# tontinton/dbeel

Hardware: AMD Instinct MI355X
Metric: compaction_MBps_input (higher is better)
Workload: dtype u8; 1 GPU; cfg3_8run_x_1GiB; n_runs=8, entries_per_run=987000, key_size=32, keep_tombstones=False, parallelism=independent_jobs_x1

## Files before the change

dbeel_amd/csrc/dbeel_gpu.hip:

```cpp
#include <cstdarg>
#include <cstdint>
#include <cstdio>
#include <cstring>
#include <cstdlib>
#include <new>
#include <vector>

#include <hip/hip_runtime.h>
#include <rocprim/rocprim.hpp>

#include "../../include/dbeel_gpu.h"

#define MAX_RUNS 64

static thread_local char g_err[512];

static void set_err(const char* fmt, ...) {
    va_list ap;
    va_start(ap, fmt);
    vsnprintf(g_err, sizeof g_err, fmt, ap);
    va_end(ap);
}

extern "C" const char* dbeel_gpu_last_error(void) { return g_err; }
// ... 113 lines not shown


#define DERR_CORRUPT 1u
#define DERR_UNSORTED 2u

__device__ __forceinline__ uint64_t key_prefix(const uint8_t* key,
                                               uint64_t klen) {
    uint64_t v = 0;
    if (klen >= 8) {
        v = ld_u64(key);
    } else {
        for (uint64_t j = 0; j < klen; j++) v |= (uint64_t)key[j] << (8 * j);
    }
    return __builtin_bswap64(v);
}

template <int KB, bool TS> struct AuxT;
template <int KB> struct AuxT<KB, false> {
    uint8_t key[KB];
    uint32_t klen;
};
template <int KB> struct AuxT<KB, true> {
    uint8_t key[KB];
    uint32_t klen;
    uint32_t rsv;
    uint64_t ts_lo;
    int64_t ts_hi;
};
static_assert(sizeof(AuxT<12, false>) == 16, "tier-0 aux must be 16B");
static_assert(sizeof(AuxT<24, true>) == 48, "tier-1 aux must be 48B");
static_assert(sizeof(AuxT<40, true>) == 64, "tier-2 aux must be 64B");

template <int KB, bool TS>
__device__ __forceinline__ int cmp_keys_sfx(const RunsDesc& R,
                                            const AuxT<KB, TS>* aux, int rA,
                                            uint64_t iA, int rB,
                                            uint64_t iB) {
    const AuxT<KB, TS>* a = aux + R.entry_base[rA] + iA;
    const AuxT<KB, TS>* b = aux + R.entry_base[rB] + iB;
    uint32_t la = a->klen, lb = b->klen;
    uint32_t n = la < lb ? la : lb;
    uint32_t ns = n > 8 ? n - 8 : 0;
    if (ns > KB) ns = KB;
    #pragma unroll
    for (uint32_t i = 0; i < KB; i += 8) {
        if (i >= ns) break;
        uint64_t va, vb;
        __builtin_memcpy(&va, a->key + i, 8);
        __builtin_memcpy(&vb, b->key + i, 8);
        if (i + 8 > ns) {
            uint64_t mask = (~0ull) >> (8 * (i + 8 - ns));
            va &= mask;
            vb &= mask;
        }
        if (va != vb) {
            va = __builtin_bswap64(va);
            vb = __builtin_bswap64(vb);
            return va < vb ? -1 : 1;
        }
    }
    if (la > (uint32_t)(8 + KB) && lb > (uint32_t)(8 + KB)) {
        EView ea, eb;
        if (!load_entry(R, rA, iA, ea) || !load_entry(R, rB, iB, eb))
            return -1;
        return cmp_keys(ea.key, ea.klen, eb.key, eb.klen);
    }
    return la < lb ? -1 : (la > lb ? 1 : 0);
}

__device__ __forceinline__ int cmp_ts_run_blob(const RunsDesc& R, int rA,
                                               uint64_t iA, int rB,
                                               uint64_t iB) {
    EView a, b;
    if (!load_entry(R, rA, iA, a) || !load_entry(R, rB, iB, b))
        return rA < rB ? -1 : 1;
    uint64_t alo, blo;
    int64_t ahi, bhi;
    load_ts(a, alo, ahi);
    load_ts(b, blo, bhi);
    if (ahi != bhi) return ahi < bhi ? -1 : 1;
    if (alo != blo) return alo < blo ? -1 : 1;
    return rA < rB ? -1 : (rA > rB ? 1 : 0);
}

template <int KB, bool TS>
__device__ __forceinline__ int cmp_sfx_full(const RunsDesc& R,
                                            const AuxT<KB, TS>* aux, int rA,
                                            uint64_t iA, int rB,
                                            uint64_t iB) {
    int c = cmp_keys_sfx<KB, TS>(R, aux, rA, iA, rB, iB);
    if (c) return c;
    if constexpr (TS) {
        const AuxT<KB, TS>* a = aux + R.entry_base[rA] + iA;
        const AuxT<KB, TS>* b = aux + R.entry_base[rB] + iB;
        if (a->ts_hi != b->ts_hi) return a->ts_hi < b->ts_hi ? -1 : 1;
        if (a->ts_lo != b->ts_lo) return a->ts_lo < b->ts_lo ? -1 : 1;
        return rA < rB ? -1 : (rA > rB ? 1 : 0);
    } else {
        return cmp_ts_run_blob(R, rA, iA, rB, iB);
    }
}

template <int KB, bool TS>
__global__ void k_prepare(RunsDesc R, uint64_t g0, uint64_t g1,
                          uint64_t* pfx, AuxT<KB, TS>* aux, uint32_t* err) {
    uint64_t stride = (uint64_t)gridDim.x * blockDim.x;
    for (uint64_t g = g0 + (uint64_t)blockIdx.x * blockDim.x + threadIdx.x;
         g < g1; g += stride) {
        int r = 0;
        while (r + 1 < R.n_runs && g >= R.entry_base[r + 1]) r++;
        uint64_t i = g - R.entry_base[r];
        EView e;
        if (!load_entry(R, r, i, e)) {
            atomicOr(err, DERR_CORRUPT);
            pfx[g] = 0;
            AuxT<KB, TS> z = {};
            aux[g] = z;
            continue;
        }
        pfx[g] = key_prefix(e.key, e.klen);
        AuxT<KB, TS> a;
        a.klen = (uint32_t)e.klen;
        if constexpr (TS) {
            a.rsv = 0;
            load_ts(e, a.ts_lo, a.ts_hi);
        }
        uint32_t nk = e.klen > 8 ? (uint32_t)e.klen - 8 : 0;
        if (nk > KB) nk = KB;
        if (nk >= KB) {
            #pragma unroll
            for (uint32_t j = 0; j < KB; j += 8) {
                uint64_t v = ld_u64(e.key + 8 + j);
                uint32_t nb = (KB - j) < 8 ? (KB - j) : 8;
                __builtin_memcpy(a.key + j, &v, nb);
            }
        } else {
            #pragma unroll
            for (uint32_t j = 0; j < KB; j += 8) {
                uint64_t v = 0;
                if (j < nk) {
                    v = ld_u64(e.key + 8 + j);
                    if (j + 8 > nk)
                        v &= (~0ull) >> (8 * (j + 8 - nk));
                }
                uint32_t nb = (KB - j) < 8 ? (KB - j) : 8;
                __builtin_memcpy(a.key + j, &v, nb);
            }
        }
        aux[g] = a;
        if (ld_u64(e.raw) != e.klen ||
            ld_u64(e.raw + 8 + e.klen) != (uint64_t)e.full_size - 32 - e.klen)
            atomicOr(err, DERR_CORRUPT);
        if (i + 1 < R.count[r]) {
            uint64_t noff = ld_u64(R.index[r] + (i + 1) * 16);
            if (e.off + e.full_size > noff)
                atomicOr(err, DERR_CORRUPT);
        }
    }
}


#define CORANK_BLOCK 256
#define CORANK_STEPS 8
#define CORANK_BLOCK_POS (CORANK_BLOCK * CORANK_STEPS)
#define CR_LOSER 0x80000000u
#define CR_MASK 0x7FFFFFFFu

struct PairDesc {
    uint32_t a, b;
    uint64_t chunk_base;
};

template <int KB, bool TS>
__global__ void k_corners(RunsDesc R, const uint64_t* pfx,
                          const AuxT<KB, TS>* aux, const PairDesc* pairs,
                          uint32_t n_pairs, uint64_t total_chunks,
                          uint64_t* corners) {
    uint64_t stride = (uint64_t)gridDim.x * blockDim.x;
    for (uint64_t t = (uint64_t)blockIdx.x * blockDim.x + threadIdx.x;
         t < total_chunks; t += stride) {
        uint32_t plo = 0, phi = n_pairs;
        while (plo < phi) {
            uint32_t mid = (plo + phi) >> 1;
            if (pairs[mid].chunk_base <= t)
                plo = mid + 1;
            else
                phi = mid;
        }
        const PairDesc P = pairs[plo - 1];
        const int a = (int)P.a, b = (int)P.b;
        const uint64_t Na = R.count[a], Nb = R.count[b];
        const uint64_t* gpa = pfx + R.entry_base[a];
        const uint64_t* gpb = pfx + R.entry_base[b];
        uint64_t diag = (t - P.chunk_base) * CORANK_BLOCK_POS;
        uint64_t slo = diag > Nb ? diag - Nb : 0;
        uint64_t shi = diag < Na ? diag : Na;
        while (slo < shi) {
            uint64_t mid = (slo + shi) >> 1;
            uint64_t pa = gpa[mid], pb = gpb[diag - mid - 1];
            int c = (pa != pb)
                        ? (pa < pb ? -1 : 1)
                        : cmp_sfx_full<KB, TS>(R, aux, a, mid, b,
                                               diag - mid - 1);
            if (c < 0)
                slo = mid + 1;
            else
                shi = mid;
        }
        corners[t] = slo;
    }
}

template <int KB, bool TS, int BLK = CORANK_BLOCK>
__global__ __launch_bounds__(BLK) void k_corank(
    RunsDesc R, const uint64_t* pfx, const AuxT<KB, TS>* aux,
    const PairDesc* pairs, uint32_t n_pairs, uint64_t total_chunks,
    const uint64_t* corners, uint32_t* cr) {
    constexpr int STEPS = CORANK_BLOCK_POS / BLK;
    __shared__ uint64_t s_pfx[CORANK_BLOCK_POS + 2];
    __shared__ uint32_t s_cr[CORANK_BLOCK_POS];
    for (uint64_t t = blockIdx.x; t < total_chunks; t += gridDim.x) {
        uint32_t plo = 0, phi = n_pairs;
        while (plo < phi) {
            uint32_t mid = (plo + phi) >> 1;
            if (pairs[mid].chunk_base <= t)
                plo = mid + 1;
            else
                phi = mid;
        }
        uint64_t pair_end_chunk =
            (plo < n_pairs) ? pairs[plo].chunk_base : total_chunks;
        const PairDesc P = pairs[plo - 1];
        const int a = (int)P.a, b = (int)P.b;
        const uint64_t Na = R.count[a], Nb = R.count[b];
        const uint64_t* gpa = pfx + R.entry_base[a];
        const uint64_t* gpb = pfx + R.entry_base[b];
        uint64_t diag0 = (t - P.chunk_base) * CORANK_BLOCK_POS;
        uint64_t diag1 = diag0 + CORANK_BLOCK_POS;
        if (diag1 > Na + Nb) diag1 = Na + Nb;

        const uint64_t iaS = corners[t];
        const uint64_t ibS = diag0 - iaS;
        const uint64_t iaE = (t + 1 < pair_end_chunk) ? corners[t + 1] : Na;
        const uint64_t ibE = diag1 - iaE;
        const uint32_t lenA = (uint32_t)(iaE - iaS);
        const uint32_t lenB = (uint32_t)(ibE - ibS);

        for (uint32_t u = threadIdx.x; u < lenA; u += BLK)
            s_pfx[u] = gpa[iaS + u];
        for (uint32_t u = threadIdx.x; u < lenB; u += BLK)
            s_pfx[lenA + u] = gpb[ibS + u];
        __syncthreads();
        const uint64_t* sA = s_pfx;
        const uint64_t* sB = s_pfx + lenA;

        uint32_t L = lenA + lenB;
        uint32_t d = threadIdx.x * STEPS;
        if (d < L) {
            uint32_t slo = d > lenB ? d - lenB : 0;
            uint32_t shi = d < lenA ? d : lenA;
            while (slo < shi) {
                uint32_t mid = (slo + shi) >> 1;
                uint64_t pa = sA[mid], pb = sB[d - mid - 1];
                int c = (pa != pb) ? (pa < pb ? -1 : 1)
                                   : cmp_sfx_full<KB, TS>(R, aux, a, iaS + mid,
                                                          b, ibS + d - mid - 1);
                if (c < 0)
                    slo = mid + 1;
                else
                    shi = mid;
            }
            uint32_t ja = slo, jb = d - slo;
            uint32_t dend = d + STEPS;
            if (dend > L) dend = L;

            for (uint32_t pos = d; pos < dend; pos++) {
                bool take_a;
                if (ja >= lenA)
                    take_a = false;
                else if (jb >= lenB)
                    take_a = true;
                else {
                    uint64_t pa = sA[ja], pb = sB[jb];
                    take_a = (pa != pb)
                                 ? (pa < pb)
                                 : (cmp_sfx_full<KB, TS>(R, aux, a, iaS + ja, b,
                                                         ibS + jb) < 0);
                }
                if (take_a) {
                    uint64_t gib = ibS + jb;
                    uint32_t v = (uint32_t)gib;
                    if (gib < Nb) {
                        uint64_t pb =
                            (jb < lenB) ? sB[jb] : gpb[gib];
                        if (pb == sA[ja] &&
                            cmp_keys_sfx<KB, TS>(R, aux, a, iaS + ja, b,
                                                 gib) == 0)
                            v |= CR_LOSER;
                    }
                    s_cr[ja] = v;
                    ja++;
                } else {
                    uint64_t gia = iaS + ja;
                    uint32_t v = (uint32_t)gia;
                    if (gia < Na) {
                        uint64_t pa =
                            (ja < lenA) ? sA[ja] : gpa[gia];
                        if (pa == sB[jb] &&
                            cmp_keys_sfx<KB, TS>(R, aux, b, ibS + jb, a,
                                                 gia) == 0)
                            v |= CR_LOSER;
                    }
                    s_cr[lenA + jb] = v;
                    jb++;
                }
            }
        }
        __syncthreads();
        {
            uint32_t al = (uint32_t)a - R.job_lo[a];
            uint32_t bl = (uint32_t)b - R.job_lo[b];
            uint32_t sa = bl < al ? bl : bl - 1;
            uint32_t sb = al < bl ? al : al - 1;
            uint32_t* cra = cr + (uint64_t)sa * R.total + R.entry_base[a] +
                            iaS;
            uint32_t* crb = cr + (uint64_t)sb * R.total + R.entry_base[b] +
                            ibS;
            for (uint32_t u = threadIdx.x; u < lenA; u += BLK)
                cra[u] = s_cr[u];
            for (uint32_t u = threadIdx.x; u < lenB; u += BLK)
                crb[u] = s_cr[lenA + u];
        }
        __syncthreads();
    }
}

struct RankRec {
    uint64_t src;
    uint32_t key_size;
    uint32_t full_size;
};
// ... 34 lines not shown
            rank += v & CR_MASK;
            winner &= !(v & CR_LOSER);
        }
        uint64_t dlen = (uint64_t)e.full_size - 32 - e.klen;
        bool keep = winner && (keep_tombstones || dlen != 0);
        RankRec m;
        m.src = ((uint64_t)r << 48) | e.off | (keep ? RR_KEEP : 0);
        m.key_size = e.key_size;
        m.full_size = e.full_size;
        rrec[rank] = m;
    }
}

#define PK_SHIFT 38
#define PK_MASK ((1ull << PK_SHIFT) - 1)
struct RankRecSize {
    __device__ uint64_t operator()(const RankRec& r) const {
        return (r.src & RR_KEEP) ? (uint64_t)r.full_size : 0ull;
    }
};
struct RankRecFlag {
    __device__ uint32_t operator()(const RankRec& r) const {
        return (r.src & RR_KEEP) ? 1u : 0u;
    }
};
struct RankRecPacked {
    __device__ uint64_t operator()(const RankRec& r) const {
        return (r.src & RR_KEEP)
                   ? ((uint64_t)r.full_size | (1ull << PK_SHIFT))
                   : 0ull;
    }
};

__global__ void k_emit(RunsDesc R, const RankRec* rrec,
                       const uint64_t* dst_off, const uint32_t* pos,
                       uint64_t total, uint8_t* out_index,
                       uint64_t* src_map) {
    uint64_t stride = (uint64_t)gridDim.x * blockDim.x;
    for (uint64_t g = (uint64_t)blockIdx.x * blockDim.x + threadIdx.x;
         g < total; g += stride) {
        RankRec m = rrec[g];
        if (!(m.src & RR_KEEP)) continue;
        uint64_t p = pos[g];
        uint8_t* rec = out_index + p * 16;
        uint64_t off = dst_off[g];
        __builtin_memcpy(rec, &off, 8);
        __builtin_memcpy(rec + 8, &m.key_size, 4);
        __builtin_memcpy(rec + 12, &m.full_size, 4);
        src_map[p] = (uint64_t)(R.data[(m.src >> 48) & 0x7FFF] +
                                (m.src & RR_OFF_MASK));
    }
}

__global__ void k_emit_packed(RunsDesc R, const RankRec* rrec,
                              const uint64_t* packed, uint64_t total,
                              uint8_t* out_index, uint64_t* src_map) {
    uint64_t stride = (uint64_t)gridDim.x * blockDim.x;
    for (uint64_t g = (uint64_t)blockIdx.x * blockDim.x + threadIdx.x;
         g < total; g += stride) {
        RankRec m = rrec[g];
        if (!(m.src & RR_KEEP)) continue;
        uint64_t v = packed[g];
        uint64_t p = v >> PK_SHIFT;
        uint8_t* rec = out_index + p * 16;
        uint64_t off = v & PK_MASK;
        __builtin_memcpy(rec, &off, 8);
        __builtin_memcpy(rec + 8, &m.key_size, 4);
        __builtin_memcpy(rec + 12, &m.full_size, 4);
        src_map[p] = (uint64_t)(R.data[(m.src >> 48) & 0x7FFF] +
                                (m.src & RR_OFF_MASK));
    }
}

#define COPY_BLOCK 256
#define COPY_WINDOW 16384
#define COPY_SPAN 516

#define COPY_GRANULES (COPY_WINDOW / 16)

__global__ void k_winmap(const uint8_t* out_index, uint64_t n_surv,
                         uint64_t total_bytes, uint32_t win,
                         uint32_t* win_p0) {
    uint64_t n_windows = (total_bytes + win - 1) / win;
    uint64_t stride = (uint64_t)gridDim.x * blockDim.x;
    for (uint64_t w = (uint64_t)blockIdx.x * blockDim.x + threadIdx.x;
         w < n_windows; w += stride) {
        uint64_t wstart = (uint64_t)w * win;
        uint64_t lo = 0, hi = n_surv;
        while (lo < hi) {
            uint64_t mid = (lo + hi) >> 1;
            if (ld_u64(out_index + mid * 16) <= wstart)
                lo = mid + 1;
            else
                hi = mid;
        }
        win_p0[w] = (uint32_t)(lo - 1);
    }
}

template <int BLK, int WIN>
__global__ __launch_bounds__(BLK) void k_copy(
    const uint8_t* out_index, const uint64_t* src_map,
    const uint32_t* win_p0, uint64_t n_surv, uint64_t total_bytes,
    uint8_t* out_data) {
    constexpr int SPAN = WIN / 32 + 4;
    constexpr int GRAN = WIN / 16;
    __shared__ uint64_t s_off[SPAN + 1];
    __shared__ uint64_t s_src[SPAN];
    __shared__ uint16_t s_gid[GRAN];

    uint64_t n_windows = (total_bytes + WIN - 1) / WIN;
    for (uint64_t w = blockIdx.x; w < n_windows; w += gridDim.x) {
        uint64_t wstart = w * WIN;
        uint64_t p0 = win_p0[w];
        uint64_t p_end = (w + 1 < n_windows) ? (uint64_t)win_p0[w + 1] + 1
                                             : n_surv;
        uint32_t cnt = (uint32_t)(p_end - p0);
        if (cnt > SPAN) cnt = SPAN;
        if (cnt > n_surv - p0) cnt = (uint32_t)(n_surv - p0);
        for (uint32_t u = threadIdx.x; u <= cnt; u += BLK) {
            uint64_t p = p0 + u;
            if (u == cnt)
                s_off[cnt] = (p < n_surv) ? ld_u64(out_index + p * 16)
                                          : total_bytes;
            else {
                s_off[u] = ld_u64(out_index + p * 16);
                s_src[u] = src_map[p];
            }
        }
        __syncthreads();
        if (cnt >= 128) {
            for (uint32_t u = threadIdx.x; u < cnt; u += BLK) {
                uint64_t b0 = s_off[u], b1 = s_off[u + 1];
                uint64_t g0 = (b0 <= wstart) ? 0 : ((b0 - wstart + 15) >> 4);
                uint64_t g1 = (b1 - wstart + 15) >> 4;
                if (g1 > GRAN) g1 = GRAN;
                for (uint64_t g = g0; g < g1; g++) s_gid[g] = (uint16_t)u;
// ... 319 lines not shown
    }
    atomicMax(&smax, m);
    __syncthreads();
    if (threadIdx.x == 0) atomicMax(out, smax);
}

struct dbeel_gpu_job {
    int device = -1;
    hipStream_t stream = nullptr;
    hipStream_t copy_stream = nullptr;
    hipEvent_t ev[8] = {};
    int prep_valid = 0;
    RunsDesc desc{};
    uint8_t* d_input = nullptr;
    bool borrowed = false;
    RankRec* d_rank = nullptr;
    uint64_t* d_dstoff = nullptr;
    uint32_t* d_pos = nullptr;
    int aux_kind = 2;
    uint8_t* d_outindex = nullptr;
    uint64_t* d_srcmap = nullptr;
    uint8_t* d_outdata = nullptr;
    void* d_scantmp = nullptr;
    size_t scantmp_bytes = 0;
    uint32_t* d_err = nullptr;
    uint64_t* d_pfx = nullptr;
    void* d_aux = nullptr;
    uint32_t* d_cr = nullptr;
    void* d_pairs = nullptr;
    uint32_t n_pairs = 0;
    uint64_t total_chunks = 0;
    uint32_t* d_winp0 = nullptr;
    uint64_t* d_corners = nullptr;
    uint64_t total_entries = 0;
    uint64_t total_data_bytes = 0;
    uint64_t input_bytes = 0;
    std::vector<uint64_t> job_gbase;
    int last_scan_packed = 0;
    uint64_t out_data_len = 0;
    uint64_t out_entries = 0;
    bool have_result = false;
    double h2d_ms = 0.0;
};

static int validate_runs(const dbeel_run_view* runs, size_t n_runs) {
    if (!runs || n_runs == 0) {
        set_err("runs is null or empty");
        return DBEEL_ERR_INVALID_ARG;
    }
    if (n_runs > MAX_RUNS) {
        set_err("n_runs %zu exceeds MAX_RUNS %d", n_runs, MAX_RUNS);
        return DBEEL_ERR_INVALID_ARG;
    }
    for (size_t r = 0; r < n_runs; r++) {
        if (runs[r].index_len % 16) {
            set_err("run %zu: index_len %zu not a multiple of 16", r,
                    runs[r].index_len);
            return DBEEL_ERR_CORRUPT;
        }
        if ((runs[r].data_len && !runs[r].data) ||
            (runs[r].index_len && !runs[r].index)) {
            set_err("run %zu: null pointer with nonzero length", r);
            return DBEEL_ERR_INVALID_ARG;
        }
        if (runs[r].data_len >= (1ull << 48)) {
            set_err("run %zu: data_len too large", r);
// ... 66 lines not shown
        total += runs[r].index_len / 16;
        total_data += runs[r].data_len;
    }
    job->total_entries = total;
    job->total_data_bytes = total_data;
    job->input_bytes = input_bytes;

#define JOB_CHECK(call)                                                     \
    do {                                                                    \
        hipError_t _e = (call);                                             \
        if (_e != hipSuccess) {                                             \
            set_err("%s failed: %s", #call, hipGetErrorString(_e));         \
            dbeel_gpu_job_destroy(job);                                     \
            return (_e == hipErrorOutOfMemory) ? DBEEL_ERR_OOM              \
                                               : DBEEL_ERR_HIP;             \
        }                                                                   \
    } while (0)

    JOB_CHECK(hipStreamCreate(&job->stream));
    for (int i = 0; i < 8; i++) JOB_CHECK(hipEventCreate(&job->ev[i]));

    if (!borrowed)
        JOB_CHECK(hipMalloc(&job->d_input,
                            (input_bytes ? input_bytes : 16) + 32));
    uint64_t n = total ? total : 1;
    JOB_CHECK(hipMalloc(&job->d_rank, n * sizeof(RankRec)));
    JOB_CHECK(hipMalloc(&job->d_dstoff, n * sizeof(uint64_t)));
    JOB_CHECK(hipMalloc(&job->d_pos, n * sizeof(uint32_t)));
    JOB_CHECK(hipMalloc(&job->d_outindex, n * 16));
    JOB_CHECK(hipMalloc(&job->d_srcmap, n * sizeof(uint64_t)));
    JOB_CHECK(hipMalloc(&job->d_outdata, total_data ? total_data : 16));
    JOB_CHECK(hipMalloc(&job->d_err, 2 * sizeof(uint32_t)));
    JOB_CHECK(hipMalloc(&job->d_pfx, n * sizeof(uint64_t)));
    uint32_t max_job_runs = 1;
    {
        for (size_t j = 0; j < n_jobs; j++)
            if (runs_per_job[j] > max_job_runs)
                max_job_runs = runs_per_job[j];
    }
    JOB_CHECK(hipMalloc(&job->d_cr,
                        (max_job_runs > 1 ? (max_job_runs - 1) * n : 1) *
                            4));
    JOB_CHECK(hipMalloc(&job->d_winp0,
                        (total_data / 8192 + 2) * sizeof(uint32_t)));

    size_t t1 = 0, t2 = 0;
    rocprim::exclusive_scan(nullptr, t1,
                            rocprim::make_transform_iterator(job->d_rank,
                                                             RankRecSize{}),
                            job->d_dstoff, (uint64_t)0, n,
                            rocprim::plus<uint64_t>(), job->stream);
    rocprim::exclusive_scan(nullptr, t2,
                            rocprim::make_transform_iterator(job->d_rank,
                                                             RankRecFlag{}),
                            job->d_pos, (uint32_t)0, n,
                            rocprim::plus<uint32_t>(), job->stream);
    job->scantmp_bytes = t1 > t2 ? t1 : t2;
    JOB_CHECK(hipMalloc(&job->d_scantmp, job->scantmp_bytes));

    JOB_CHECK(hipEventRecord(job->ev[0], job->stream));
    uint8_t* p = borrowed ? nullptr : job->d_input + 16;
    RunsDesc& D = job->desc;
    memset(&D, 0, sizeof D);
    D.n_runs = (int)n_runs;
    D.total = total;
    {
// ... 196 lines not shown
        free(out->index);
        memset(out, 0, sizeof *out);
        set_err("fetch_job D2H failed: %s", hipGetErrorString(ce));
        return DBEEL_ERR_HIP;
    }
    for (uint64_t i = 0; i < nsurv; i++) {
        uint64_t o = ld_u64_host(out->index + i * 16) - off0;
        memcpy(out->index + i * 16, &o, 8);
    }
    out->data_len = dlen;
    out->index_len = nsurv * 16;
    out->entries_written = nsurv;
    return DBEEL_OK;
}

extern "C" void dbeel_gpu_job_destroy(dbeel_gpu_job* job) {
    if (!job) return;
    if (job->device >= 0) hipSetDevice(job->device);
    hipFree(job->d_input);
    hipFree(job->d_rank);
    hipFree(job->d_dstoff);
    hipFree(job->d_pos);
    hipFree(job->d_outindex);
    hipFree(job->d_srcmap);
    hipFree(job->d_outdata);
    hipFree(job->d_scantmp);
    hipFree(job->d_err);
    hipFree(job->d_pfx);
    hipFree(job->d_aux);
    hipFree(job->d_cr);
    hipFree(job->d_pairs);
    hipFree(job->d_winp0);
    hipFree(job->d_corners);
    for (int i = 0; i < 8; i++)
        if (job->ev[i]) hipEventDestroy(job->ev[i]);
    if (job->stream) hipStreamDestroy(job->stream);
    if (job->copy_stream) hipStreamDestroy(job->copy_stream);
    delete job;
}


extern "C" int dbeel_gpu_pin_host(const void* ptr, size_t len) {
    g_err[0] = 0;
    if (!ptr || !len) {
        set_err("pin_host: null/empty buffer");
        return DBEEL_ERR_INVALID_ARG;
    }
    hipError_t e = hipHostRegister(const_cast<void*>(ptr), len,
                                   hipHostRegisterDefault);
    if (e == hipErrorHostMemoryAlreadyRegistered) return DBEEL_OK;
    if (e != hipSuccess) {
        set_err("hipHostRegister failed: %s", hipGetErrorString(e));
        return DBEEL_ERR_HIP;
    }
    return DBEEL_OK;
}

extern "C" int dbeel_gpu_unpin_host(const void* ptr) {
    g_err[0] = 0;
    hipError_t e = hipHostUnregister(const_cast<void*>(ptr));
    if (e != hipSuccess && e != hipErrorHostMemoryNotRegistered) {
        set_err("hipHostUnregister failed: %s", hipGetErrorString(e));
        return DBEEL_ERR_HIP;
    }
    return DBEEL_OK;
}
// ... 179 lines not shown
        set_err("corrupt entry/index record in streamed ingest");
        return DBEEL_ERR_CORRUPT;
    }

    if (stats) {
        float copy_ms = 0, prep_ms = 0, wall_ms = 0;
        (void)hipEventElapsedTime(&copy_ms, ev_cs0, ev_cs1);
        (void)hipEventElapsedTime(&prep_ms, ev_ks0, ev_ks1);
        (void)hipEventElapsedTime(&wall_ms, ev_cs0, ev_ks1);
        if (prep_ms > wall_ms) wall_ms = prep_ms;
        stats->ingest_ms = wall_ms;
        stats->copy_ms = copy_ms;
        stats->prep_ms = prep_ms;
        stats->bytes = job->input_bytes;
        stats->chunks = total_chunks;
    }
    job->h2d_ms = 0.0;
    job->prep_valid = 1;
    cleanup();
    return DBEEL_OK;
#undef ING_CHECK
}

static uint32_t pick_grid(uint64_t work_items, uint32_t block) {
    uint64_t blocks = (work_items + block - 1) / block;
    if (blocks > 2048) blocks = 2048;
    if (blocks == 0) blocks = 1;
    return (uint32_t)blocks;
}


static void launch_copy(hipStream_t s, const uint8_t* out_index,
                        const uint64_t* src_map, uint32_t* win_p0,
                        uint64_t n_surv, uint64_t total_out,
                        uint8_t* out_data) {
    int variant = -1;
    if (const char* v = getenv("DBEEL_COPY_VARIANT")) variant = atoi(v);
    uint64_t gcap = 0;
    if (const char* g = getenv("DBEEL_COPY_GRID")) {
        long v = atol(g);
        if (v >= 64) gcap = (uint64_t)v;
    }
    if (variant < 0) {
        uint64_t avg = n_surv ? total_out / n_surv : 0;
        if (avg > 2048) {
            variant = 0;
            if (!gcap) gcap = 16384;
        } else if (avg >= 512) {
            variant = 4;
        } else {
            variant = 3;
            if (!gcap) gcap = 16384;
        }
    }
    if (!gcap) gcap = 4096;
    uint32_t win = (variant == 1)   ? 8192
                   : (variant == 3) ? 32768
                   : (variant == 4) ? 65536
                                    : 16384;
    uint32_t blk = (variant >= 2) ? 512 : 256;
    uint64_t windows = (total_out + win - 1) / win;
    uint32_t grid = windows > gcap ? (uint32_t)gcap : (uint32_t)windows;
    hipLaunchKernelGGL(k_winmap, dim3(pick_grid(windows, 256)), dim3(256),
                       0, s, out_index, n_surv, total_out, win, win_p0);
    void (*kc)(const uint8_t*, const uint64_t*, const uint32_t*, uint64_t,
               uint64_t, uint8_t*) = k_copy<256, 16384>;
    if (variant == 1) kc = k_copy<256, 8192>;
    if (variant == 2) kc = k_copy<512, 16384>;
    if (variant == 3) kc = k_copy<512, 32768>;
    if (variant == 4) kc = k_copy<512, 65536>;
    hipLaunchKernelGGL(kc, dim3(grid), dim3(blk), 0, s, out_index, src_map,
                       win_p0, n_surv, total_out, out_data);
}

extern "C" int dbeel_gpu_job_run(dbeel_gpu_job* job, int keep_tombstones,
                                 uint64_t* out_data_len,
                                 uint64_t* out_entries,
                                 dbeel_compact_timings* t) {
    g_err[0] = 0;
    if (!job) {
        set_err("job is null");
        return DBEEL_ERR_INVALID_ARG;
    }
    HIP_CHECK(hipSetDevice(job->device));
    hipStream_t s = job->stream;
    uint64_t n = job->total_entries;
    job->have_result = false;

    int skip_prep = job->prep_valid;
    HIP_CHECK(hipMemsetAsync(job->d_err, 0, 2 * sizeof(uint32_t), s));

    HIP_CHECK(hipEventRecord(job->ev[0], s));
    if (n) {
        uint32_t grid = pick_grid(n, 256);
        uint64_t cgrid = job->total_chunks;
        if (cgrid > 16384) cgrid = 16384;
        int corank_wide = 0;
        if (const char* w = getenv("DBEEL_CORANK_BLOCK"))
            corank_wide = atoi(w) >= 512;
        switch (job->aux_kind) {
#define STAGE1(KB, TS)                                                      \
    case (KB == 12 ? 0 : (KB == 24 ? 1 : 2)):                               \
        if (!skip_prep)                                                     \
            hipLaunchKernelGGL((k_prepare<KB, TS>), dim3(grid), dim3(256),  \
                               0, s, job->desc, (uint64_t)0, n, job->d_pfx, \
// ... 43 lines not shown
    if (const char* m = getenv("DBEEL_SCAN_MODE")) {
        if (!strcmp(m, "two")) packed = false;
    }
    if (n) {
        size_t tmp = job->scantmp_bytes;
        if (packed) {
            (void)rocprim::exclusive_scan(
                job->d_scantmp, tmp,
                rocprim::make_transform_iterator(job->d_rank,
                                                 RankRecPacked{}),
                job->d_dstoff, (uint64_t)0, n, rocprim::plus<uint64_t>(),
                s);
        } else {
            (void)rocprim::exclusive_scan(
                job->d_scantmp, tmp,
                rocprim::make_transform_iterator(job->d_rank,
                                                 RankRecSize{}),
                job->d_dstoff, (uint64_t)0, n, rocprim::plus<uint64_t>(),
                s);
            tmp = job->scantmp_bytes;
            (void)rocprim::exclusive_scan(
                job->d_scantmp, tmp,
                rocprim::make_transform_iterator(job->d_rank,
                                                 RankRecFlag{}),
                job->d_pos, (uint32_t)0, n, rocprim::plus<uint32_t>(), s);
        }
    }
    HIP_CHECK(hipEventRecord(job->ev[2], s));
    if (n) {
        uint32_t grid = pick_grid(n, 256);
        if (packed)
            hipLaunchKernelGGL(k_emit_packed, dim3(grid), dim3(256), 0, s,
                               job->desc, job->d_rank, job->d_dstoff, n,
                               job->d_outindex, job->d_srcmap);
        else
            hipLaunchKernelGGL(k_emit, dim3(grid), dim3(256), 0, s,
                               job->desc, job->d_rank, job->d_dstoff,
                               job->d_pos, n, job->d_outindex,
                               job->d_srcmap);
    }
    HIP_CHECK(hipEventRecord(job->ev[3], s));

    RankRec last_rec = {};
    uint64_t last_off = 0;
    uint32_t last_pos = 0;
    uint32_t err = 0;
    if (n) {
        HIP_CHECK(hipMemcpyAsync(&last_rec, job->d_rank + (n - 1), 16,
                                 hipMemcpyDeviceToHost, s));
        HIP_CHECK(hipMemcpyAsync(&last_off, job->d_dstoff + (n - 1), 8,
                                 hipMemcpyDeviceToHost, s));
        if (!packed)
            HIP_CHECK(hipMemcpyAsync(&last_pos, job->d_pos + (n - 1), 4,
                                     hipMemcpyDeviceToHost, s));
    }
    HIP_CHECK(hipMemcpyAsync(&err, job->d_err, 4, hipMemcpyDeviceToHost, s));
    HIP_CHECK(hipStreamSynchronize(s));
    if (err) {
        set_err(err & DERR_UNSORTED
                    ? "input run not strictly sorted by unique keys "
                      "(dbeel flush invariant violated)"
                    : "corrupt entry/index record");
        return DBEEL_ERR_CORRUPT;
    }
    if (packed) {
        last_pos = (uint32_t)(last_off >> PK_SHIFT);
        last_off &= PK_MASK;
    }
    job->last_scan_packed = packed ? 1 : 0;
    uint64_t last_kept = (n && (last_rec.src & RR_KEEP)) ? 1 : 0;
    uint64_t total_out = last_off + (last_kept ? last_rec.full_size : 0);
    uint64_t n_surv = (uint64_t)last_pos + last_kept;

    HIP_CHECK(hipEventRecord(job->ev[4], s));
    if (total_out)
        launch_copy(s, job->d_outindex, job->d_srcmap, job->d_winp0,
                    n_surv, total_out, job->d_outdata);
    HIP_CHECK(hipEventRecord(job->ev[5], s));
    HIP_CHECK(hipStreamSynchronize(s));
    HIP_CHECK(hipGetLastError());

    job->out_data_len = total_out;
    job->out_entries = n_surv;
    job->have_result = true;
    if (out_data_len) *out_data_len = total_out;
    if (out_entries) *out_entries = n_surv;
    if (t) {
        float prep_ms = 0, rank_ms = 0, scan_ms = 0, emit_ms = 0,
              copy_ms = 0;
        (void)hipEventElapsedTime(&prep_ms, job->ev[0], job->ev[6]);
        (void)hipEventElapsedTime(&rank_ms, job->ev[6], job->ev[1]);
        (void)hipEventElapsedTime(&scan_ms, job->ev[1], job->ev[2]);
        (void)hipEventElapsedTime(&emit_ms, job->ev[2], job->ev[3]);
        (void)hipEventElapsedTime(&copy_ms, job->ev[4], job->ev[5]);
        t->h2d_ms = job->h2d_ms;
        t->prep_ms = prep_ms;
        t->rank_ms = rank_ms;
        t->scan_ms = scan_ms;
        t->emit_ms = emit_ms;
        t->copy_ms = copy_ms;
        t->kernel_ms = prep_ms + rank_ms + scan_ms + emit_ms + copy_ms;
        t->d2h_ms = 0.0;
    }
    return DBEEL_OK;
}


__device__ __forceinline__ uint64_t d_mix64(uint64_t h) {
    h ^= h >> 30;
    h *= 0xbf58476d1ce4e5b9ull;
    h ^= h >> 27;
    h *= 0x94d049bb133111ebull;
    h ^= h >> 31;
// ... 1273 lines not shown
    if (e == hipSuccess && end_key_len)
        e = hipMemcpyAsync(d_kb + start_key_len, end_key, end_key_len,
                           hipMemcpyHostToDevice, s);
    if (e == hipSuccess)
        e = hipMalloc(&d_ranges, (n_ranges ? 2 * n_ranges : 1) * 4);
    if (e == hipSuccess && n_ranges) {
        e = hipMemcpyAsync(d_ranges, range_starts, n_ranges * 4,
                           hipMemcpyHostToDevice, s);
        if (e == hipSuccess)
            e = hipMemcpyAsync(d_ranges + n_ranges, range_ends,
                               n_ranges * 4, hipMemcpyHostToDevice, s);
    }
    if (e == hipSuccess)
        e = hipMemsetAsync(job->d_err, 0, 8, s);
    if (e == hipSuccess && n) {
        hipLaunchKernelGGL(k_scanflag, dim3(pick_grid(n, 256)), dim3(256),
                           0, s, job->desc, d_kb, (uint64_t)start_key_len,
                           (uint64_t)end_key_len, start_key ? 1 : 0,
                           end_key ? 1 : 0, d_ranges,
                           d_ranges + n_ranges, (uint32_t)n_ranges,
                           job->d_rank, job->d_err);
        size_t tmp = job->scantmp_bytes;
        (void)rocprim::exclusive_scan(
            job->d_scantmp, tmp,
            rocprim::make_transform_iterator(job->d_rank, RankRecSize{}),
            job->d_dstoff, (uint64_t)0, n, rocprim::plus<uint64_t>(), s);
        tmp = job->scantmp_bytes;
        (void)rocprim::exclusive_scan(
            job->d_scantmp, tmp,
            rocprim::make_transform_iterator(job->d_rank, RankRecFlag{}),
            job->d_pos, (uint32_t)0, n, rocprim::plus<uint32_t>(), s);
        hipLaunchKernelGGL(k_emit, dim3(pick_grid(n, 256)), dim3(256), 0,
                           s, job->desc, job->d_rank, job->d_dstoff,
                           job->d_pos, n, job->d_outindex, job->d_srcmap);
    }
    RankRec last_rec = {};
    uint64_t last_off = 0;
    uint32_t last_pos = 0, derr = 0;
    if (e == hipSuccess && n) {
        e = hipMemcpyAsync(&last_rec, job->d_rank + (n - 1), 16,
                           hipMemcpyDeviceToHost, s);
        if (e == hipSuccess)
            e = hipMemcpyAsync(&last_off, job->d_dstoff + (n - 1), 8,
                               hipMemcpyDeviceToHost, s);
        if (e == hipSuccess)
            e = hipMemcpyAsync(&last_pos, job->d_pos + (n - 1), 4,
                               hipMemcpyDeviceToHost, s);
    }
    if (e == hipSuccess)
        e = hipMemcpyAsync(&derr, job->d_err, 4, hipMemcpyDeviceToHost, s);
    if (e == hipSuccess) e = hipStreamSynchronize(s);
    if (e == hipSuccess) e = hipGetLastError();

    job->last_scan_packed = 0;
    int ret = DBEEL_OK;
    if (e != hipSuccess) {
        set_err("scan failed: %s", hipGetErrorString(e));
        ret = DBEEL_ERR_HIP;
    } else if (derr) {
        set_err("corrupt entry/index record");
        ret = DBEEL_ERR_CORRUPT;
    } else {
        uint64_t last_kept = (n && (last_rec.src & RR_KEEP)) ? 1 : 0;
        uint64_t total_out =
            last_off + (last_kept ? last_rec.full_size : 0);
        uint64_t n_surv = (uint64_t)last_pos + last_kept;
        if (total_out)
            launch_copy(s, job->d_outindex, job->d_srcmap, job->d_winp0,
                        n_surv, total_out, job->d_outdata);
        e = hipStreamSynchronize(s);
        if (e == hipSuccess) e = hipGetLastError();
        if (e != hipSuccess) {
            set_err("scan copy failed: %s", hipGetErrorString(e));
            ret = DBEEL_ERR_HIP;
        } else {
            job->out_data_len = total_out;
            job->out_entries = n_surv;
            job->have_result = true;
            ret = dbeel_gpu_job_fetch(job, out);
        }
    }
    hipFree(d_kb);
    hipFree(d_ranges);
    dbeel_gpu_job_destroy(job);
    return ret;
}

extern "C" int dbeel_gpu_compact_timed(const dbeel_run_view* runs,
                                       size_t n_runs, int keep_tombstones,
                                       int device, dbeel_compact_result* out,
                                       dbeel_compact_timings* t) {
    if (!out) {
        set_err("out is null");
        return DBEEL_ERR_INVALID_ARG;
    }
    dbeel_gpu_job* job = nullptr;
    int rc = dbeel_gpu_job_create(runs, n_runs, device, &job);
    if (rc) return rc;
    rc = dbeel_gpu_job_run(job, keep_tombstones, nullptr, nullptr, t);
    if (!rc) rc = dbeel_gpu_job_fetch(job, out);
    dbeel_gpu_job_destroy(job);
    return rc;
}

extern "C" int dbeel_gpu_compact(const dbeel_run_view* runs, size_t n_runs,
                                 int keep_tombstones, int device,
                                 dbeel_compact_result* out) {
    return dbeel_gpu_compact_timed(runs, n_runs, keep_tombstones, device, out,
                                   nullptr);
}


static int host_key_cmp(const uint8_t* a, uint64_t la, const uint8_t* b,
// ... 182 lines not shown
```

Before: 2.398 million MB/s.

## Compute totals on device, drop mid-pipeline host sync, and batch corank tie resolution

Output totals (bytes, survivor count, error flag) are now written by the emit kernel into a device struct. The copy kernels read that struct directly, so the host no longer synchronises and reads back values before launching the copy, and the whole job finishes with a single stream sync. The copy grid is sized from the input byte total, an upper bound, so some workgroups may find no work. Separately, the corank merge prefetches aux records for the first prefix tie in each step and precomputes its result. The diagonal search also narrows full comparisons to the range of equal prefixes, cutting dependent loads on the tie path.

After: 2.502 million MB/s (median of 6 runs). 4.3% higher.

```diff
diff --git a/dbeel_amd/csrc/dbeel_gpu.hip b/dbeel_amd/csrc/dbeel_gpu.hip
--- a/dbeel_amd/csrc/dbeel_gpu.hip
+++ b/dbeel_amd/csrc/dbeel_gpu.hip
@@ -169,13 +169,11 @@
 static_assert(sizeof(AuxT<40, true>) == 64, "tier-2 aux must be 64B");
 
 template <int KB, bool TS>
-__device__ __forceinline__ int cmp_keys_sfx(const RunsDesc& R,
-                                            const AuxT<KB, TS>* aux, int rA,
-                                            uint64_t iA, int rB,
-                                            uint64_t iB) {
-    const AuxT<KB, TS>* a = aux + R.entry_base[rA] + iA;
-    const AuxT<KB, TS>* b = aux + R.entry_base[rB] + iB;
-    uint32_t la = a->klen, lb = b->klen;
+__device__ __forceinline__ int cmp_keys_rec(const AuxT<KB, TS>& a,
+                                            const AuxT<KB, TS>& b,
+                                            bool& deep) {
+    deep = false;
+    uint32_t la = a.klen, lb = b.klen;
     uint32_t n = la < lb ? la : lb;
     uint32_t ns = n > 8 ? n - 8 : 0;
     if (ns > KB) ns = KB;
@@ -183,8 +181,8 @@
     for (uint32_t i = 0; i < KB; i += 8) {
         if (i >= ns) break;
         uint64_t va, vb;
-        __builtin_memcpy(&va, a->key + i, 8);
-        __builtin_memcpy(&vb, b->key + i, 8);
+        __builtin_memcpy(&va, a.key + i, 8);
+        __builtin_memcpy(&vb, b.key + i, 8);
         if (i + 8 > ns) {
             uint64_t mask = (~0ull) >> (8 * (i + 8 - ns));
             va &= mask;
@@ -197,12 +195,28 @@
         }
     }
     if (la > (uint32_t)(8 + KB) && lb > (uint32_t)(8 + KB)) {
+        deep = true;
+        return 0;
+    }
+    return la < lb ? -1 : (la > lb ? 1 : 0);
+}
+
+template <int KB, bool TS>
+__device__ __forceinline__ int cmp_keys_sfx(const RunsDesc& R,
+                                            const AuxT<KB, TS>* aux, int rA,
+                                            uint64_t iA, int rB,
+                                            uint64_t iB) {
+    const AuxT<KB, TS>* a = aux + R.entry_base[rA] + iA;
+    const AuxT<KB, TS>* b = aux + R.entry_base[rB] + iB;
+    bool deep;
+    int c = cmp_keys_rec<KB, TS>(*a, *b, deep);
+    if (deep) {
         EView ea, eb;
         if (!load_entry(R, rA, iA, ea) || !load_entry(R, rB, iB, eb))
             return -1;
         return cmp_keys(ea.key, ea.klen, eb.key, eb.klen);
     }
-    return la < lb ? -1 : (la > lb ? 1 : 0);
+    return c;
 }
 
 __device__ __forceinline__ int cmp_ts_run_blob(const RunsDesc& R, int rA,
@@ -236,6 +250,62 @@
     } else {
         return cmp_ts_run_blob(R, rA, iA, rB, iB);
     }
+}
+
+template <int KB, bool TS>
+__device__ __forceinline__ bool tie_eval(const RunsDesc& R,
+                                         const AuxT<KB, TS>* aux, int rA,
+                                         uint64_t iA, int rB, uint64_t iB,
+                                         bool& keq) {
+    int c = cmp_keys_sfx<KB, TS>(R, aux, rA, iA, rB, iB);
+    keq = (c == 0);
+    if (c) return c < 0;
+    if constexpr (TS) {
+        const AuxT<KB, TS>* a = aux + R.entry_base[rA] + iA;
+        const AuxT<KB, TS>* b = aux + R.entry_base[rB] + iB;
+        if (a->ts_hi != b->ts_hi) return a->ts_hi < b->ts_hi;
+        if (a->ts_lo != b->ts_lo) return a->ts_lo < b->ts_lo;
+        return rA < rB;
+    } else {
+        return cmp_ts_run_blob(R, rA, iA, rB, iB) < 0;
+    }
+}
+
+template <typename T, typename PA, typename PB, typename FULL>
+__device__ __forceinline__ T diag_split(T lo, T hi, T d, PA pa, PB pb,
+                                        FULL full_lt) {
+    const T hi0 = hi;
+    while (lo < hi) {
+        T mid = (lo + hi) >> 1;
+        if (pa(mid) < pb(d - mid - 1))
+            lo = mid + 1;
+        else
+            hi = mid;
+    }
+    if (lo < hi0 && pa(lo) == pb(d - lo - 1)) {
+        T e = lo + 1;
+        if (e < hi0 && pa(e) == pb(d - e - 1)) {
+            T l = e + 1, h = hi0;
+            while (l < h) {
+                T m = (l + h) >> 1;
+                if (pa(m) == pb(d - m - 1))
+                    l = m + 1;
+                else
+                    h = m;
+            }
+            e = l;
+        }
+        T l = lo, h = e;
+        while (l < h) {
+            T m = (l + h) >> 1;
+            if (full_lt(m, d - m - 1))
+                l = m + 1;
+            else
+                h = m;
+        }
+        lo = l;
+    }
+    return lo;
 }
 
 template <int KB, bool TS>
@@ -300,6 +370,9 @@
 #define CORANK_BLOCK 256
 #define CORANK_STEPS 8
 #define CORANK_BLOCK_POS (CORANK_BLOCK * CORANK_STEPS)
+#ifndef CORANK_TIE_HINTS
+#define CORANK_TIE_HINTS 1
+#endif
 #define CR_LOSER 0x80000000u
 #define CR_MASK 0x7FFFFFFFu
 
@@ -332,18 +405,12 @@
         uint64_t diag = (t - P.chunk_base) * CORANK_BLOCK_POS;
         uint64_t slo = diag > Nb ? diag - Nb : 0;
         uint64_t shi = diag < Na ? diag : Na;
-        while (slo < shi) {
-            uint64_t mid = (slo + shi) >> 1;
-            uint64_t pa = gpa[mid], pb = gpb[diag - mid - 1];
-            int c = (pa != pb)
-                        ? (pa < pb ? -1 : 1)
-                        : cmp_sfx_full<KB, TS>(R, aux, a, mid, b,
-                                               diag - mid - 1);
-            if (c < 0)
-                slo = mid + 1;
-            else
-                shi = mid;
-        }
+        slo = diag_split<uint64_t>(
+            slo, shi, diag, [&](uint64_t s) { return gpa[s]; },
+            [&](uint64_t s) { return gpb[s]; },
+            [&](uint64_t s, uint64_t u) {
+                return cmp_sfx_full<KB, TS>(R, aux, a, s, b, u) < 0;
+            });
         corners[t] = slo;
     }
 }
@@ -396,41 +463,105 @@
         if (d < L) {
             uint32_t slo = d > lenB ? d - lenB : 0;
             uint32_t shi = d < lenA ? d : lenA;
-            while (slo < shi) {
-                uint32_t mid = (slo + shi) >> 1;
-                uint64_t pa = sA[mid], pb = sB[d - mid - 1];
-                int c = (pa != pb) ? (pa < pb ? -1 : 1)
-                                   : cmp_sfx_full<KB, TS>(R, aux, a, iaS + mid,
-                                                          b, ibS + d - mid - 1);
-                if (c < 0)
-                    slo = mid + 1;
-                else
-                    shi = mid;
-            }
+            slo = diag_split<uint32_t>(
+                slo, shi, d, [&](uint32_t s) { return sA[s]; },
+                [&](uint32_t s) { return sB[s]; },
+                [&](uint32_t s, uint32_t u) {
+                    return cmp_sfx_full<KB, TS>(R, aux, a, iaS + s, b,
+                                                ibS + u) < 0;
+                });
             uint32_t ja = slo, jb = d - slo;
             uint32_t dend = d + STEPS;
             if (dend > L) dend = L;
 
+            constexpr int M = CORANK_TIE_HINTS;
+            uint32_t hx[M], hy[M];
+            uint32_t hbits = 0;
+            #pragma unroll
+            for (int m = 0; m < M; m++) hx[m] = hy[m] = ~0u;
+            {
+                uint32_t nh = 0, x = ja, y = jb, c = d;
+                while (c < dend && x < lenA && y < lenB && nh < M) {
+                    uint64_t pa = sA[x], pb = sB[y];
+                    if (pa < pb) {
+                        x++, c++;
+                    } else if (pa > pb) {
+                        y++, c++;
+                    } else {
+                        #pragma unroll
+                        for (int m = 0; m < M; m++)
+                            if ((int)nh == m) hx[m] = x, hy[m] = y;
+                        nh++, x++, y++, c += 2;
+                    }
+                }
+                const AuxT<KB, TS>* xa = aux + R.entry_base[a] + iaS;
+                const AuxT<KB, TS>* xb = aux + R.entry_base[b] + ibS;
+                AuxT<KB, TS> ra[M], rb[M];
+                #pragma unroll
+                for (int m = 0; m < M; m++)
+                    if (m < (int)nh) {
+                        ra[m] = xa[hx[m]];
+                        rb[m] = xb[hy[m]];
+                    }
+                #pragma unroll
+                for (int m = 0; m < M; m++)
+                    if (m < (int)nh) {
+                        bool deep;
+                        int k = cmp_keys_rec<KB, TS>(ra[m], rb[m], deep);
+                        bool first = k < 0;
+                        if (k == 0 && !deep) {
+                            if constexpr (TS) {
+                                first = ra[m].ts_hi != rb[m].ts_hi
+                                            ? ra[m].ts_hi < rb[m].ts_hi
+                                        : ra[m].ts_lo != rb[m].ts_lo
+                                            ? ra[m].ts_lo < rb[m].ts_lo
+                                            : a < b;
+                            } else {
+                                first = cmp_ts_run_blob(R, a, iaS + hx[m], b,
+                                                        ibS + hy[m]) < 0;
+                            }
+                        }
+                        if (!deep)
+                            hbits |= (1u | (k == 0 ? 2u : 0u) |
+                                      (first ? 4u : 0u)) << (3 * m);
+                    }
+            }
+
             for (uint32_t pos = d; pos < dend; pos++) {
                 bool take_a;
+                bool both = false;
+                bool keq = false;
                 if (ja >= lenA)
                     take_a = false;
                 else if (jb >= lenB)
                     take_a = true;
                 else {
+                    both = true;
                     uint64_t pa = sA[ja], pb = sB[jb];
-                    take_a = (pa != pb)
-                                 ? (pa < pb)
-                                 : (cmp_sfx_full<KB, TS>(R, aux, a, iaS + ja, b,
-                                                         ibS + jb) < 0);
+                    if (pa != pb) {
+                        take_a = pa < pb;
+                    } else {
+                        uint32_t h = 0;
+                        #pragma unroll
+                        for (int m = 0; m < M; m++)
+                            if (hx[m] == ja && hy[m] == jb)
+                                h = hbits >> (3 * m);
+                        if (h & 1u) {
+                            keq = h & 2u;
+                            take_a = h & 4u;
+                        } else {
+                            take_a = tie_eval<KB, TS>(R, aux, a, iaS + ja, b,
+                                                      ibS + jb, keq);
+                        }
+                    }
                 }
                 if (take_a) {
                     uint64_t gib = ibS + jb;
                     uint32_t v = (uint32_t)gib;
-                    if (gib < Nb) {
-                        uint64_t pb =
-                            (jb < lenB) ? sB[jb] : gpb[gib];
-                        if (pb == sA[ja] &&
+                    if (both) {
+                        if (keq) v |= CR_LOSER;
+                    } else if (gib < Nb) {
+                        if (gpb[gib] == sA[ja] &&
                             cmp_keys_sfx<KB, TS>(R, aux, a, iaS + ja, b,
                                                  gib) == 0)
                             v |= CR_LOSER;
@@ -440,10 +571,10 @@
                 } else {
                     uint64_t gia = iaS + ja;
                     uint32_t v = (uint32_t)gia;
-                    if (gia < Na) {
-                        uint64_t pa =
-                            (ja < lenA) ? sA[ja] : gpa[gia];
-                        if (pa == sB[jb] &&
+                    if (both) {
+                        if (keq) v |= CR_LOSER;
+                    } else if (gia < Na) {
+                        if (gpa[gia] == sB[jb] &&
                             cmp_keys_sfx<KB, TS>(R, aux, b, ibS + jb, a,
                                                  gia) == 0)
                             v |= CR_LOSER;
@@ -544,14 +675,35 @@
     }
 };
 
+struct StepTotals {
+    uint64_t total_out;
+    uint64_t n_surv;
+    uint64_t err;
+};
+
+__device__ __forceinline__ void store_totals(StepTotals* tot,
+                                             const uint32_t* err,
+                                             const RankRec& last,
+                                             uint64_t last_off,
+                                             uint64_t last_pos) {
+    uint32_t e = *err;
+    uint64_t kept = (last.src & RR_KEEP) ? 1 : 0;
+    tot->total_out = e ? 0 : last_off + (kept ? last.full_size : 0);
+    tot->n_surv = e ? 0 : last_pos + kept;
+    tot->err = e;
+}
+
 __global__ void k_emit(RunsDesc R, const RankRec* rrec,
                        const uint64_t* dst_off, const uint32_t* pos,
                        uint64_t total, uint8_t* out_index,
-                       uint64_t* src_map) {
+                       uint64_t* src_map, const uint32_t* err,
+                       StepTotals* tot) {
     uint64_t stride = (uint64_t)gridDim.x * blockDim.x;
     for (uint64_t g = (uint64_t)blockIdx.x * blockDim.x + threadIdx.x;
          g < total; g += stride) {
         RankRec m = rrec[g];
+        if (g + 1 == total)
+            store_totals(tot, err, m, dst_off[g], pos[g]);
         if (!(m.src & RR_KEEP)) continue;
         uint64_t p = pos[g];
         uint8_t* rec = out_index + p * 16;
@@ -566,11 +718,15 @@
 
 __global__ void k_emit_packed(RunsDesc R, const RankRec* rrec,
                               const uint64_t* packed, uint64_t total,
-                              uint8_t* out_index, uint64_t* src_map) {
+                              uint8_t* out_index, uint64_t* src_map,
+                              const uint32_t* err, StepTotals* tot) {
     uint64_t stride = (uint64_t)gridDim.x * blockDim.x;
     for (uint64_t g = (uint64_t)blockIdx.x * blockDim.x + threadIdx.x;
          g < total; g += stride) {
         RankRec m = rrec[g];
+        if (g + 1 == total)
+            store_totals(tot, err, m, packed[g] & PK_MASK,
+                         packed[g] >> PK_SHIFT);
         if (!(m.src & RR_KEEP)) continue;
         uint64_t v = packed[g];
         uint64_t p = v >> PK_SHIFT;
@@ -590,9 +746,9 @@
 
 #define COPY_GRANULES (COPY_WINDOW / 16)
 
-__global__ void k_winmap(const uint8_t* out_index, uint64_t n_surv,
-                         uint64_t total_bytes, uint32_t win,
-                         uint32_t* win_p0) {
+__global__ void k_winmap(const uint8_t* out_index, const StepTotals* tot,
+                         uint32_t win, uint32_t* win_p0) {
+    const uint64_t n_surv = tot->n_surv, total_bytes = tot->total_out;
     uint64_t n_windows = (total_bytes + win - 1) / win;
     uint64_t stride = (uint64_t)gridDim.x * blockDim.x;
     for (uint64_t w = (uint64_t)blockIdx.x * blockDim.x + threadIdx.x;
@@ -613,8 +769,8 @@
 template <int BLK, int WIN>
 __global__ __launch_bounds__(BLK) void k_copy(
     const uint8_t* out_index, const uint64_t* src_map,
-    const uint32_t* win_p0, uint64_t n_surv, uint64_t total_bytes,
-    uint8_t* out_data) {
+    const uint32_t* win_p0, const StepTotals* tot, uint8_t* out_data) {
+    const uint64_t n_surv = tot->n_surv, total_bytes = tot->total_out;
     constexpr int SPAN = WIN / 32 + 4;
     constexpr int GRAN = WIN / 16;
     __shared__ uint64_t s_off[SPAN + 1];
@@ -1000,6 +1156,8 @@
     uint64_t total_chunks = 0;
     uint32_t* d_winp0 = nullptr;
     uint64_t* d_corners = nullptr;
+    StepTotals* d_tot = nullptr;
+    StepTotals* h_tot = nullptr;
     uint64_t total_entries = 0;
     uint64_t total_data_bytes = 0;
     uint64_t input_bytes = 0;
@@ -1132,6 +1290,8 @@
     JOB_CHECK(hipMalloc(&job->d_outdata, total_data ? total_data : 16));
     JOB_CHECK(hipMalloc(&job->d_err, 2 * sizeof(uint32_t)));
     JOB_CHECK(hipMalloc(&job->d_pfx, n * sizeof(uint64_t)));
+    JOB_CHECK(hipMalloc(&job->d_tot, sizeof(StepTotals)));
+    JOB_CHECK(hipHostMalloc(&job->h_tot, sizeof(StepTotals)));
     uint32_t max_job_runs = 1;
     {
         for (size_t j = 0; j < n_jobs; j++)
@@ -1394,6 +1554,8 @@
     hipFree(job->d_pairs);
     hipFree(job->d_winp0);
     hipFree(job->d_corners);
+    hipFree(job->d_tot);
+    if (job->h_tot) hipHostFree(job->h_tot);
     for (int i = 0; i < 8; i++)
         if (job->ev[i]) hipEventDestroy(job->ev[i]);
     if (job->stream) hipStreamDestroy(job->stream);
@@ -1639,8 +1801,8 @@
 
 static void launch_copy(hipStream_t s, const uint8_t* out_index,
                         const uint64_t* src_map, uint32_t* win_p0,
-                        uint64_t n_surv, uint64_t total_out,
-                        uint8_t* out_data) {
+                        const StepTotals* tot, uint64_t in_entries,
+                        uint64_t in_bytes, uint8_t* out_data) {
     int variant = -1;
     if (const char* v = getenv("DBEEL_COPY_VARIANT")) variant = atoi(v);
     uint64_t gcap = 0;
@@ -1649,7 +1811,7 @@
         if (v >= 64) gcap = (uint64_t)v;
     }
     if (variant < 0) {
-        uint64_t avg = n_surv ? total_out / n_surv : 0;
+        uint64_t avg = in_entries ? in_bytes / in_entries : 0;
         if (avg > 2048) {
             variant = 0;
             if (!gcap) gcap = 16384;
@@ -1666,18 +1828,19 @@
                    : (variant == 4) ? 65536
                                     : 16384;
     uint32_t blk = (variant >= 2) ? 512 : 256;
-    uint64_t windows = (total_out + win - 1) / win;
+    uint64_t windows = (in_bytes + win - 1) / win;
+    if (!windows) return;
     uint32_t grid = windows > gcap ? (uint32_t)gcap : (uint32_t)windows;
     hipLaunchKernelGGL(k_winmap, dim3(pick_grid(windows, 256)), dim3(256),
-                       0, s, out_index, n_surv, total_out, win, win_p0);
-    void (*kc)(const uint8_t*, const uint64_t*, const uint32_t*, uint64_t,
-               uint64_t, uint8_t*) = k_copy<256, 16384>;
+                       0, s, out_index, tot, win, win_p0);
+    void (*kc)(const uint8_t*, const uint64_t*, const uint32_t*,
+               const StepTotals*, uint8_t*) = k_copy<256, 16384>;
     if (variant == 1) kc = k_copy<256, 8192>;
     if (variant == 2) kc = k_copy<512, 16384>;
     if (variant == 3) kc = k_copy<512, 32768>;
     if (variant == 4) kc = k_copy<512, 65536>;
     hipLaunchKernelGGL(kc, dim3(grid), dim3(blk), 0, s, out_index, src_map,
-                       win_p0, n_surv, total_out, out_data);
+                       win_p0, tot, out_data);
 }
 
 extern "C" int dbeel_gpu_job_run(dbeel_gpu_job* job, int keep_tombstones,
@@ -1787,30 +1950,28 @@
         if (packed)
             hipLaunchKernelGGL(k_emit_packed, dim3(grid), dim3(256), 0, s,
                                job->desc, job->d_rank, job->d_dstoff, n,
-                               job->d_outindex, job->d_srcmap);
+                               job->d_outindex, job->d_srcmap, job->d_err,
+                               job->d_tot);
         else
             hipLaunchKernelGGL(k_emit, dim3(grid), dim3(256), 0, s,
                                job->desc, job->d_rank, job->d_dstoff,
                                job->d_pos, n, job->d_outindex,
-                               job->d_srcmap);
+                               job->d_srcmap, job->d_err, job->d_tot);
+    } else {
+        HIP_CHECK(hipMemsetAsync(job->d_tot, 0, sizeof(StepTotals), s));
     }
     HIP_CHECK(hipEventRecord(job->ev[3], s));
 
-    RankRec last_rec = {};
-    uint64_t last_off = 0;
-    uint32_t last_pos = 0;
-    uint32_t err = 0;
-    if (n) {
-        HIP_CHECK(hipMemcpyAsync(&last_rec, job->d_rank + (n - 1), 16,
-                                 hipMemcpyDeviceToHost, s));
-        HIP_CHECK(hipMemcpyAsync(&last_off, job->d_dstoff + (n - 1), 8,
-                                 hipMemcpyDeviceToHost, s));
-        if (!packed)
-            HIP_CHECK(hipMemcpyAsync(&last_pos, job->d_pos + (n - 1), 4,
-                                     hipMemcpyDeviceToHost, s));
-    }
-    HIP_CHECK(hipMemcpyAsync(&err, job->d_err, 4, hipMemcpyDeviceToHost, s));
+    HIP_CHECK(hipEventRecord(job->ev[4], s));
+    if (n)
+        launch_copy(s, job->d_outindex, job->d_srcmap, job->d_winp0,
+                    job->d_tot, n, job->total_data_bytes, job->d_outdata);
+    HIP_CHECK(hipEventRecord(job->ev[5], s));
+    HIP_CHECK(hipMemcpyAsync(job->h_tot, job->d_tot, sizeof(StepTotals),
+                             hipMemcpyDeviceToHost, s));
     HIP_CHECK(hipStreamSynchronize(s));
+    HIP_CHECK(hipGetLastError());
+    uint32_t err = (uint32_t)job->h_tot->err;
     if (err) {
         set_err(err & DERR_UNSORTED
                     ? "input run not strictly sorted by unique keys "
@@ -1818,22 +1979,9 @@
                     : "corrupt entry/index record");
         return DBEEL_ERR_CORRUPT;
     }
-    if (packed) {
-        last_pos = (uint32_t)(last_off >> PK_SHIFT);
-        last_off &= PK_MASK;
-    }
     job->last_scan_packed = packed ? 1 : 0;
-    uint64_t last_kept = (n && (last_rec.src & RR_KEEP)) ? 1 : 0;
-    uint64_t total_out = last_off + (last_kept ? last_rec.full_size : 0);
-    uint64_t n_surv = (uint64_t)last_pos + last_kept;
-
-    HIP_CHECK(hipEventRecord(job->ev[4], s));
-    if (total_out)
-        launch_copy(s, job->d_outindex, job->d_srcmap, job->d_winp0,
-                    n_surv, total_out, job->d_outdata);
-    HIP_CHECK(hipEventRecord(job->ev[5], s));
-    HIP_CHECK(hipStreamSynchronize(s));
-    HIP_CHECK(hipGetLastError());
+    uint64_t total_out = job->h_tot->total_out;
+    uint64_t n_surv = job->h_tot->n_surv;
 
     job->out_data_len = total_out;
     job->out_entries = n_surv;
@@ -3173,23 +3321,16 @@
             job->d_pos, (uint32_t)0, n, rocprim::plus<uint32_t>(), s);
         hipLaunchKernelGGL(k_emit, dim3(pick_grid(n, 256)), dim3(256), 0,
                            s, job->desc, job->d_rank, job->d_dstoff,
-                           job->d_pos, n, job->d_outindex, job->d_srcmap);
-    }
-    RankRec last_rec = {};
-    uint64_t last_off = 0;
-    uint32_t last_pos = 0, derr = 0;
-    if (e == hipSuccess && n) {
-        e = hipMemcpyAsync(&last_rec, job->d_rank + (n - 1), 16,
+                           job->d_pos, n, job->d_outindex, job->d_srcmap,
+                           job->d_err, job->d_tot);
+        launch_copy(s, job->d_outindex, job->d_srcmap, job->d_winp0,
+                    job->d_tot, n, job->total_data_bytes, job->d_outdata);
+    } else if (e == hipSuccess) {
+        e = hipMemsetAsync(job->d_tot, 0, sizeof(StepTotals), s);
+    }
+    if (e == hipSuccess)
+        e = hipMemcpyAsync(job->h_tot, job->d_tot, sizeof(StepTotals),
                            hipMemcpyDeviceToHost, s);
-        if (e == hipSuccess)
-            e = hipMemcpyAsync(&last_off, job->d_dstoff + (n - 1), 8,
-                               hipMemcpyDeviceToHost, s);
-        if (e == hipSuccess)
-            e = hipMemcpyAsync(&last_pos, job->d_pos + (n - 1), 4,
-                               hipMemcpyDeviceToHost, s);
-    }
-    if (e == hipSuccess)
-        e = hipMemcpyAsync(&derr, job->d_err, 4, hipMemcpyDeviceToHost, s);
     if (e == hipSuccess) e = hipStreamSynchronize(s);
     if (e == hipSuccess) e = hipGetLastError();
 
@@ -3198,28 +3339,14 @@
     if (e != hipSuccess) {
         set_err("scan failed: %s", hipGetErrorString(e));
         ret = DBEEL_ERR_HIP;
-    } else if (derr) {
+    } else if (job->h_tot->err) {
         set_err("corrupt entry/index record");
         ret = DBEEL_ERR_CORRUPT;
     } else {
-        uint64_t last_kept = (n && (last_rec.src & RR_KEEP)) ? 1 : 0;
-        uint64_t total_out =
-            last_off + (last_kept ? last_rec.full_size : 0);
-        uint64_t n_surv = (uint64_t)last_pos + last_kept;
-        if (total_out)
-            launch_copy(s, job->d_outindex, job->d_srcmap, job->d_winp0,
-                        n_surv, total_out, job->d_outdata);
-        e = hipStreamSynchronize(s);
-        if (e == hipSuccess) e = hipGetLastError();
-        if (e != hipSuccess) {
-            set_err("scan copy failed: %s", hipGetErrorString(e));
-            ret = DBEEL_ERR_HIP;
-        } else {
-            job->out_data_len = total_out;
-            job->out_entries = n_surv;
-            job->have_result = true;
-            ret = dbeel_gpu_job_fetch(job, out);
-        }
+        job->out_data_len = job->h_tot->total_out;
+        job->out_entries = job->h_tot->n_surv;
+        job->have_result = true;
+        ret = dbeel_gpu_job_fetch(job, out);
     }
     hipFree(d_kb);
     hipFree(d_ranges);
```
